# zhiyuan-yang/MILE

Hardware: AMD Instinct MI355X
Metric: MCLMC integrator particle-steps/s (integrator-steps/s x ensemble size) (higher is better)
Workload: dtype f32; 1 GPU; B2: airfoil-shaped N=1052 F=5, FCN hidden_structure [64,64,64,2] relu, Gaussian head, StandardNormal prior, d=8834; ensemble_per_gpu=128, ensemble_total=128, n_thinning=10, integrator=isokinetic McLachlan, O-step-O refresh, 2 full-batch gradients/step, noise=Philox4x32-10 counter RNG, grad_kernel=mfma_w64_bf16x3, parallelism=particles sharded 128/GPU x 1, no collective (one rank, no process group), finite=True

## Files before the change

### mile_amd/csrc/mile_update.h

```cpp
#pragma once
#include <cstdlib>

#include "mile_device.h"

enum : int32_t {
  UPD_FROM_SLABS = 1 << 0,
  UPD_START = 1 << 1,
  UPD_B1 = 1 << 2,
  UPD_OA = 1 << 3,
  UPD_RECORD = 1 << 4,
  UPD_OB = 1 << 5,
  UPD_B2 = 1 << 6,
  UPD_A = 1 << 7,
  UPD_TUNE = 1 << 8,
  UPD_NO_G = 1 << 9,
};

struct UpdParams {
  int32_t d, E, S, flags;
  int32_t dp;
  int32_t prior;
  float prior_loc, prior_scale;
  float *x, *u, *g, *logp;
  const float *slabs, *llpart;
  const float *eps, *L, *sdc;
  const float *zA, *zB;
  uint64_t seed;
  const int32_t *pids;
  uint32_t stepA, stageA, stepB, stageB;
  float coef_b1, coef_b2, coef_a;
  float hA, hB;
  float *dK, *lold;
  float *out_sample;
  float *out_info;
  const float *x_in, *u_in, *g_in, *logp_in;
  float *t_eps;
  float *t_eps_max, *t_time, *t_xavg;
  float *t_W;
  float *t_avg;
  const float *bk_x, *bk_u, *bk_g, *bk_logp;
  float t_mask;
  float t_var;
  float t_trust, t_decay;
  float *upart;
  float *u_rec;
  float *x_acc;
  int32_t force_restart;
  float *nz_A, *nz_B;
  uint32_t nz_stepA, nz_stageA, nz_stepB, nz_stageB;
#ifdef MILE_LAB_UPD_EDGES
  long long *dbg_buf;
#endif
};
#ifdef MILE_LAB_UPD_EDGES
#define UPD_EDGE(k) asm volatile("s_memtime %0\n\ts_waitcnt lgkmcnt(0)" : "=s"(upd_edge[k])::"memory");
#define UPD_EDGE_WAIT asm volatile("s_waitcnt vmcnt(0)" ::: "memory");
#else
#define UPD_EDGE(k)
#define UPD_EDGE_WAIT
#endif

struct Chain {
  float M[4][4];
  float c[4];
  __device__ __forceinline__ float norm() const {
    float s = 0.0f;
#pragma unroll
    for (int a = 0; a < 4; ++a)
#pragma unroll
      for (int b = 0; b < 4; ++b) s = fmaf(c[a] * M[a][b], c[b], s);
    return sqrtf(s);
  }
  __device__ __forceinline__ float B(float eps, float coef, float gnorm, int d) {
    float ue = 0.0f;
#pragma unroll
    for (int a = 0; a < 4; ++a) ue = fmaf(c[a], M[a][1], ue);
    const float delta = eps * coef * gnorm / (float)(d - 1);
    const float omz = -expm1f(-delta);
    const float zeta = 1.0f - omz;
    const float beta = omz * (1.0f + zeta + ue * omz);
#pragma unroll
    for (int a = 0; a < 4; ++a) c[a] *= 2.0f * zeta;
    c[1] += beta;
    const float n = norm();
    if (n > 1e-13f)
#pragma unroll
      for (int a = 0; a < 4; ++a) c[a] /= n;
    return (float)(d - 1) * (delta + log1pf(0.5f * (1.0f - ue) * expm1f(-2.0f * delta)));
  }
  __device__ __forceinline__ void O(int k, float hstep, float L, int d) {
    const float nu = sqrtf(expm1f(2.0f * hstep / L) / (float)d);
    c[k] += nu;
    const float n = norm();
#pragma unroll
    for (int a = 0; a < 4; ++a) c[a] /= n;
  }
};


struct GradNorm {
  float gn, ign, ee;
  bool zero_e;
};
__device__ __forceinline__ GradNorm grad_norm(float gg) {
  GradNorm r;
  r.gn = sqrtf(gg);
  const bool ok = r.gn > 1e-13f;
  r.zero_e = ok && isinf(r.gn);
  r.ign = ok ? 1.0f / r.gn : 1.0f;
  r.ee = ok ? (r.zero_e ? 0.0f : 1.0f) : gg;
  return r;
}
__device__ __forceinline__ void chain_gram(Chain &ch, const float *S, const GradNorm &gnm) {
  const float ig = gnm.ign;
  ch.M[0][0] = S[0]; ch.M[0][1] = gnm.zero_e ? 0.0f : S[1] * ig; ch.M[0][2] = S[3]; ch.M[0][3] = S[6];
  ch.M[1][1] = gnm.ee; ch.M[1][2] = gnm.zero_e ? 0.0f : S[4] * ig; ch.M[1][3] = gnm.zero_e ? 0.0f : S[7] * ig;
  ch.M[2][2] = S[5]; ch.M[2][3] = S[9];
  ch.M[3][3] = S[8];
#pragma unroll
  for (int a = 0; a < 4; ++a)
#pragma unroll
    for (int b = 0; b < 4; ++b)
      if (b < a) ch.M[a][b] = ch.M[b][a];
  ch.c[0] = 1.0f; ch.c[1] = ch.c[2] = ch.c[3] = 0.0f;
}
__device__ __forceinline__ float nan_to_num(float v) {
  constexpr float FMAX = 3.4028234663852886e38f;
  return isnan(v) ? 0.0f : fminf(fmaxf(v, -FMAX), FMAX);
}

#define UPD_NT 1024
#define UPD_NW (UPD_NT / 64)
#define UPD_NSUM 12
#define UPD_QMAX 4

template <bool CACHED>
static __global__ __launch_bounds__(UPD_NT) void k_update(const UpdParams p) {
  __shared__ float red[UPD_NW][UPD_NSUM + 1];
  __shared__ float tot[UPD_NSUM + 1];
  const int tid = threadIdx.x, e = blockIdx.x, d = p.d;
  const size_t base = (size_t)e * d;
  const int nq = (d + 3) >> 2;
  const bool from_slabs = p.flags & UPD_FROM_SLABS;
  const bool useA = p.flags & UPD_OA, useB = p.flags & UPD_OB;
  const uint32_t pid = p.pids ? (uint32_t)p.pids[e] : (uint32_t)e;
  const float *sl = p.slabs + (size_t)e * p.S * p.dp;
  constexpr int NK = CACHED ? UPD_QMAX : 1;
  f32x4 cx[NK], cu[NK], cg[NK], ca[NK], cb[NK];

  float sm[UPD_NSUM];
#pragma unroll
  for (int k = 0; k < UPD_NSUM; ++k) sm[k] = 0.0f;
  auto pass1 = [&](int q, f32x4 &X, f32x4 &U, f32x4 &G, f32x4 &A, f32x4 &B) {
    A = f32x4{0, 0, 0, 0}; B = f32x4{0, 0, 0, 0};
    if (useA && !p.zA) A = philox_normal4(q, pid, p.stepA, p.stageA, p.seed);
    if (useB && !p.zB) B = philox_normal4(q, pid, p.stepB, p.stageB, p.seed);
#pragma unroll
    for (int m = 0; m < 4; ++m) {
      const int i = 4 * q + m;
      X[m] = U[m] = G[m] = 0.0f;
      if (i < d) {
        float gi;
        const float xi = p.x[base + i];
        if (from_slabs) {
          gi = 0.0f;
          for (int s = 0; s < p.S; ++s) gi += sl[(size_t)s * p.dp + i];
          const float t = (xi - p.prior_loc) / p.prior_scale;
          if (p.prior == MILE_PRIOR_NORMAL) {
            gi -= t / p.prior_scale;
            sm[10] = fmaf(-0.5f * t, t, sm[10]);
          } else {
            gi -= (t > 0.0f ? 1.0f : (t < 0.0f ? -1.0f : 0.0f)) / p.prior_scale;
            sm[10] -= fabsf(t);
          }
          p.g[base + i] = gi;
        } else {
          gi = p.g[base + i];
        }
        const float gs = p.sdc ? gi * p.sdc[base + i] : gi;
        const float ui = p.u[base + i];
        if (useA && p.zA) A[m] = p.zA[base + i];
        if (useB && p.zB) B[m] = p.zB[base + i];
        const float a = A[m], b = B[m];
        X[m] = xi; U[m] = ui; G[m] = gs;
        sm[0] = fmaf(ui, ui, sm[0]); sm[1] = fmaf(ui, gs, sm[1]); sm[2] = fmaf(gs, gs, sm[2]);
        sm[3] = fmaf(ui, a, sm[3]); sm[4] = fmaf(gs, a, sm[4]); sm[5] = fmaf(a, a, sm[5]);
        sm[6] = fmaf(ui, b, sm[6]); sm[7] = fmaf(gs, b, sm[7]); sm[8] = fmaf(b, b, sm[8]);
        sm[9] = fmaf(a, b, sm[9]);
      } else {
        A[m] = B[m] = 0.0f;
      }
    }
  };
  if (CACHED) {
#pragma unroll
    for (int k = 0; k < NK; ++k) {
      const int q = tid + k * UPD_NT;
      if (q < nq) pass1(q, cx[k], cu[k], cg[k], ca[k], cb[k]);
    }
  } else {
    for (int q = tid; q < nq; q += UPD_NT) pass1(q, cx[0], cu[0], cg[0], ca[0], cb[0]);
  }
#pragma unroll
  for (int k = 0; k < UPD_NSUM; ++k) sm[k] = wave_sum(sm[k]);
  if ((tid & 63) == 0)
#pragma unroll
    for (int k = 0; k < UPD_NSUM; ++k) red[tid >> 6][k] = sm[k];
  __syncthreads();
  if (tid < UPD_NSUM) {
    float t = 0.0f;
#pragma unroll
    for (int w = 0; w < UPD_NW; ++w) t += red[w][tid];
    tot[tid] = t;
  }
  __syncthreads();

  float S[UPD_NSUM];
#pragma unroll
  for (int k = 0; k < UPD_NSUM; ++k) S[k] = tot[k];
  const float eps = p.eps[e], L = p.L[e];
  float logp_now;
  if (from_slabs) {
    float ll = 0.0f;
    for (int s = 0; s < p.S; ++s) ll += p.llpart[(size_t)e * p.S + s];
    const float cst = p.prior == MILE_PRIOR_NORMAL ? -(float)d * (logf(p.prior_scale) + 0.91893853320467274f)
                                                   : -(float)d * logf(2.0f * p.prior_scale);
    logp_now = ll + (S[10] + cst);
  } else {
    logp_now = p.logp[e];
  }
  const GradNorm gnm = grad_norm(S[2]);
  const float gn = gnm.gn, ign = gnm.ign;
  Chain ch;
  chain_gram(ch, S, gnm);

  float dk = (p.flags & UPD_START) ? 0.0f : p.dK[e];
  float lold = (p.flags & UPD_START) ? logp_now : p.lold[e];
  if (p.flags & UPD_B1) dk += ch.B(eps, p.coef_b1, gn, d);
  if (p.flags & UPD_OA) ch.O(2, p.hA * eps, L, d);
  float info_dk = 0.0f, info_de = 0.0f;
  if (p.flags & UPD_RECORD) {
    info_dk = dk;
    info_de = dk - (logp_now - lold);
    dk = 0.0f;
    lold = logp_now;
  }
  if (p.flags & UPD_OB) ch.O(3, p.hB * eps, L, d);
  if (p.flags & UPD_B2) dk += ch.B(eps, p.coef_b2, gn, d);
  __syncthreads();
  if (tid == 0) {
    p.dK[e] = dk;
    p.lold[e] = lold;
    if (from_slabs) p.logp[e] = logp_now;
    if ((p.flags & UPD_RECORD) && p.out_info) {
      p.out_info[3 * e + 0] = logp_now;
      p.out_info[3 * e + 1] = info_dk;
      p.out_info[3 * e + 2] = info_de;
    }
  }
  const bool any_op = p.flags & (UPD_B1 | UPD_OA | UPD_OB | UPD_B2);
  if (!any_op && !(p.flags & UPD_A) && !p.out_sample) return;

  const float c0 = ch.c[0], c1 = ch.c[1] * ign, c2 = ch.c[2], c3 = ch.c[3];
  const float ea = eps * p.coef_a;
  auto pass2 = [&](int q, const f32x4 &X, const f32x4 &U, const f32x4 &G, const f32x4 &A, const f32x4 &B) {
#pragma unroll
    for (int m = 0; m < 4; ++m) {
      const int i = 4 * q + m;
      if (i < d) {
        const float sd = p.sdc ? p.sdc[base + i] : 1.0f;
        float v = U[m];
        if (any_op) {
          v = fmaf(c0, v, fmaf(c1, G[m], fmaf(c2, A[m], c3 * B[m])));
          p.u[base + i] = v;
        }
        if (p.out_sample) p.out_sample[base + i] = X[m];
        if (p.flags & UPD_A) p.x[base + i] = fmaf(ea * sd, v, X[m]);
      }
    }
  };
  if (CACHED) {
#pragma unroll
    for (int k = 0; k < NK; ++k) {
      const int q = tid + k * UPD_NT;
      if (q < nq) pass2(q, cx[k], cu[k], cg[k], ca[k], cb[k]);
    }
  } else {
    for (int q = tid; q < nq; q += UPD_NT) {
      f32x4 X, U, G, A = {0, 0, 0, 0}, B = {0, 0, 0, 0};
      if (useA && !p.zA) A = philox_normal4(q, pid, p.stepA, p.stageA, p.seed);
      if (useB && !p.zB) B = philox_normal4(q, pid, p.stepB, p.stageB, p.seed);
#pragma unroll
      for (int m = 0; m < 4; ++m) {
        const int i = 4 * q + m;
        X[m] = U[m] = G[m] = 0.0f;
        if (i < d) {
          X[m] = p.x[base + i]; U[m] = p.u[base + i];
          G[m] = p.g[base + i] * (p.sdc ? p.sdc[base + i] : 1.0f);
          if (useA && p.zA) A[m] = p.zA[base + i];
          if (useB && p.zB) B[m] = p.zB[base + i];
        }
      }
      pass2(q, X, U, G, A, B);
    }
  }
}

#define UPD_SEG 8192
template <int PHASE>
static __global__ __launch_bounds__(UPD_NT) void k_update_seg(const UpdParams p, float *upart, int nseg) {
  __shared__ float red[UPD_NW][UPD_NSUM + 1];
  __shared__ float tot[UPD_NSUM + 1];
  const int tid = threadIdx.x, seg = blockIdx.x, e = blockIdx.y, d = p.d;
  const size_t base = (size_t)e * d;
  const int q0 = seg * (UPD_SEG / 4), q1 = min((d + 3) >> 2, q0 + UPD_SEG / 4);
  const bool from_slabs = p.flags & UPD_FROM_SLABS;
  const bool useA = p.flags & UPD_OA, useB = p.flags & UPD_OB;
  const uint32_t pid = p.pids ? (uint32_t)p.pids[e] : (uint32_t)e;
  const float *sl = p.slabs + (size_t)e * p.S * p.dp;
  float *mine = upart + ((size_t)e * nseg + seg) * UPD_NSUM;
  if constexpr (PHASE == 1) {
    float sm[UPD_NSUM];
#pragma unroll
    for (int k = 0; k < UPD_NSUM; ++k) sm[k] = 0.0f;
    for (int q = q0 + tid; q < q1; q += UPD_NT) {
      f32x4 A = {0, 0, 0, 0}, B = {0, 0, 0, 0};
      if (useA && !p.zA) A = philox_normal4(q, pid, p.stepA, p.stageA, p.seed);
      if (useB && !p.zB) B = philox_normal4(q, pid, p.stepB, p.stageB, p.seed);
#pragma unroll
      for (int m = 0; m < 4; ++m) {
        const int i = 4 * q + m;
        if (i < d) {
          float gi;
          const float xi = p.x[base + i];
          if (from_slabs) {
            gi = 0.0f;
            for (int s = 0; s < p.S; ++s) gi += sl[(size_t)s * p.dp + i];
            const float t = (xi - p.prior_loc) / p.prior_scale;
            if (p.prior == MILE_PRIOR_NORMAL) {
              gi -= t / p.prior_scale;
              sm[10] = fmaf(-0.5f * t, t, sm[10]);
            } else {
              gi -= (t > 0.0f ? 1.0f : (t < 0.0f ? -1.0f : 0.0f)) / p.prior_scale;
              sm[10] -= fabsf(t);
            }
            p.g[base + i] = gi;
          } else {
            gi = p.g[base + i];
          }
          const float gs = p.sdc ? gi * p.sdc[base + i] : gi;
          const float ui = p.u[base + i];
          const float a = (useA && p.zA) ? p.zA[base + i] : A[m], b = (useB && p.zB) ? p.zB[base + i] : B[m];
          sm[0] = fmaf(ui, ui, sm[0]); sm[1] = fmaf(ui, gs, sm[1]); sm[2] = fmaf(gs, gs, sm[2]);
          sm[3] = fmaf(ui, a, sm[3]); sm[4] = fmaf(gs, a, sm[4]); sm[5] = fmaf(a, a, sm[5]);
          sm[6] = fmaf(ui, b, sm[6]); sm[7] = fmaf(gs, b, sm[7]); sm[8] = fmaf(b, b, sm[8]);
          sm[9] = fmaf(a, b, sm[9]);
        }
      }
    }
#pragma unroll
    for (int k = 0; k < UPD_NSUM; ++k) sm[k] = wave_sum(sm[k]);
    if ((tid & 63) == 0)
#pragma unroll
      for (int k = 0; k < UPD_NSUM; ++k) red[tid >> 6][k] = sm[k];
    __syncthreads();
    if (tid < UPD_NSUM) {
      float t = 0.0f;
#pragma unroll
      for (int w = 0; w < UPD_NW; ++w) t += red[w][tid];
      mine[tid] = t;
    }
    return;
  } else {
    if (tid < UPD_NSUM) {
      float t = 0.0f;
      for (int sg = 0; sg < nseg; ++sg) t += upart[((size_t)e * nseg + sg) * UPD_NSUM + tid];
      tot[tid] = t;
    }
    __syncthreads();
    float S[UPD_NSUM];
#pragma unroll
    for (int k = 0; k < UPD_NSUM; ++k) S[k] = tot[k];
    const float eps = p.eps[e], L = p.L[e];
    float logp_now;
    if (from_slabs) {
      float ll = 0.0f;
      for (int s = 0; s < p.S; ++s) ll += p.llpart[(size_t)e * p.S + s];
      const float cst = p.prior == MILE_PRIOR_NORMAL ? -(float)d * (logf(p.prior_scale) + 0.91893853320467274f)
                                                     : -(float)d * logf(2.0f * p.prior_scale);
      logp_now = ll + (S[10] + cst);
    } else {
      logp_now = p.logp[e];
    }
    const GradNorm gnm = grad_norm(S[2]);
    const float gn = gnm.gn, ign = gnm.ign;
    Chain ch;
    chain_gram(ch, S, gnm);
    float dk = (p.flags & UPD_START) ? 0.0f : p.dK[e];
    float lold = (p.flags & UPD_START) ? logp_now : p.lold[e];
    if (p.flags & UPD_B1) dk += ch.B(eps, p.coef_b1, gn, d);
    if (p.flags & UPD_OA) ch.O(2, p.hA * eps, L, d);
    float info_dk = 0.0f, info_de = 0.0f;
    if (p.flags & UPD_RECORD) {
      info_dk = dk;
      info_de = dk - (logp_now - lold);
      dk = 0.0f;
      lold = logp_now;
    }
    if (p.flags & UPD_OB) ch.O(3, p.hB * eps, L, d);
    if (p.flags & UPD_B2) dk += ch.B(eps, p.coef_b2, gn, d);
    const bool any_op = p.flags & (UPD_B1 | UPD_OA | UPD_OB | UPD_B2);
    if (seg == 0 && tid == 0) {
      float *st = upart + ((size_t)gridDim.y * nseg) * UPD_NSUM + (size_t)e * 8;
      st[0] = dk; st[1] = lold; st[2] = logp_now; st[3] = info_dk; st[4] = info_de;
    }
    if (!any_op && !(p.flags & UPD_A) && !p.out_sample) return;
    const float c0 = ch.c[0], c1 = ch.c[1] * ign, c2 = ch.c[2], c3 = ch.c[3];
    const float ea = eps * p.coef_a;
    for (int q = q0 + tid; q < q1; q += UPD_NT) {
      f32x4 A = {0, 0, 0, 0}, B = {0, 0, 0, 0};
      if (useA && !p.zA) A = philox_normal4(q, pid, p.stepA, p.stageA, p.seed);
      if (useB && !p.zB) B = philox_normal4(q, pid, p.stepB, p.stageB, p.seed);
#pragma unroll
      for (int m = 0; m < 4; ++m) {
        const int i = 4 * q + m;
        if (i < d) {
          const float sd = p.sdc ? p.sdc[base + i] : 1.0f;
          const float X = p.x[base + i], G = p.g[base + i] * sd;
          const float a = (useA && p.zA) ? p.zA[base + i] : A[m], b = (useB && p.zB) ? p.zB[base + i] : B[m];
          float v = p.u[base + i];
          if (any_op) {
            v = fmaf(c0, v, fmaf(c1, G, fmaf(c2, a, c3 * b)));
            p.u[base + i] = v;
          }
          if (p.out_sample) p.out_sample[base + i] = X;
          if (p.flags & UPD_A) p.x[base + i] = fmaf(ea * sd, v, X);
        }
      }
    }
  }
}
static __global__ __launch_bounds__(256) void k_update_seg_scalars(const UpdParams p, const float *upart, int nseg, int E) {
  const int e = blockIdx.x * 256 + threadIdx.x;
  if (e >= E) return;
  const float *st = upart + ((size_t)E * nseg) * UPD_NSUM + (size_t)e * 8;
  p.dK[e] = st[0];
  p.lold[e] = st[1];
  if (p.flags & UPD_FROM_SLABS) p.logp[e] = st[2];
  if ((p.flags & UPD_RECORD) && p.out_info) {
    p.out_info[3 * e + 0] = st[2];
    p.out_info[3 * e + 1] = st[3];
    p.out_info[3 * e + 2] = st[4];
  }
}

template <int AL>
__device__ __forceinline__ f32x4 ld4(const float *q) {
  if constexpr (AL == 4) {
    return *(const f32x4 *)q;
  } else if constexpr (AL == 2) {
    const f32x2 a = *(const f32x2 *)q, b = *(const f32x2 *)(q + 2);
    return f32x4{a[0], a[1], b[0], b[1]};
  } else {
    return f32x4{q[0], q[1], q[2], q[3]};
  }
}
template <int AL>
__device__ __forceinline__ void st4(float *q, const f32x4 v) {
  if constexpr (AL == 4) {
    *(f32x4 *)q = v;
  } else if constexpr (AL == 2) {
    *(f32x2 *)q = f32x2{v[0], v[1]};
    *(f32x2 *)(q + 2) = f32x2{v[2], v[3]};
  } else {
    q[0] = v[0]; q[1] = v[1]; q[2] = v[2]; q[3] = v[3];
  }
}

typedef uint32_t upd_u32x4 __attribute__((ext_vector_type(4)));
template <int AL, bool COH>
__device__ __forceinline__ f32x4 ld4_slab(const float *row, __amdgpu_buffer_rsrc_t rs, int float_off) {
  if constexpr (COH) {
    return __builtin_bit_cast(f32x4, __builtin_amdgcn_raw_buffer_load_b128(rs, float_off * 4, 0, 16));
  } else {
    return ld4<AL>(row + float_off);
  }
}
template <bool COH>
__device__ __forceinline__ float ld1_shared(const float *q) {
  if constexpr (COH) return __hip_atomic_load(q, __ATOMIC_RELAXED, __HIP_MEMORY_SCOPE_AGENT);
  else return *q;
}

template <int CF>
__host__ __device__ constexpr bool upd_needs(int k) {
  if (CF < 0) return true;
  const bool a = (CF & UPD_OA) != 0, b = (CF & UPD_OB) != 0;
  return k < 3 ? true : k < 6 ? a : k < 9 ? b : k == 9 ? (a && b) : k == 10 ? (CF & UPD_FROM_SLABS) != 0 : (CF & UPD_TUNE) != 0;
}
template <int CF>
__device__ __forceinline__ void upd_add_sums(float (&sm)[UPD_NSUM], float ui, float gs, float a, float b) {
  sm[0] = fmaf(ui, ui, sm[0]); sm[1] = fmaf(ui, gs, sm[1]); sm[2] = fmaf(gs, gs, sm[2]);
  if constexpr (upd_needs<CF>(3)) { sm[3] = fmaf(ui, a, sm[3]); sm[4] = fmaf(gs, a, sm[4]); sm[5] = fmaf(a, a, sm[5]); }
  if constexpr (upd_needs<CF>(6)) { sm[6] = fmaf(ui, b, sm[6]); sm[7] = fmaf(gs, b, sm[7]); sm[8] = fmaf(b, b, sm[8]); }
  if constexpr (upd_needs<CF>(9)) sm[9] = fmaf(a, b, sm[9]);
}

#define UPD_KIND_MID (UPD_FROM_SLABS | UPD_B1 | UPD_A | UPD_NO_G)
#define UPD_KIND_REC (UPD_FROM_SLABS | UPD_B1 | UPD_OA | UPD_RECORD | UPD_OB | UPD_B2 | UPD_A | UPD_NO_G)
#define UPD_KIND_TUNE (UPD_FROM_SLABS | UPD_B1 | UPD_OA | UPD_RECORD | UPD_TUNE | UPD_OB | UPD_B2 | UPD_A)
template <int NK, int AL, bool SDC, bool COH, int CF = -1, bool BIG = false>
__device__ __forceinline__ bool upd_fast_body(const UpdParams &p, const int e, const int tid, const int nt,
                                              float (*red)[UPD_NSUM + 1], float *bc, f32x4 *gl = nullptr) {
  const int d = p.d;
  const int flags = CF >= 0 ? CF : p.flags;
#ifdef MILE_LAB_UPD_EDGES
  unsigned long long upd_edge[10] = {}, upd_rt0, upd_rt1;
  asm volatile("s_memrealtime %0\n\ts_waitcnt lgkmcnt(0)" : "=s"(upd_rt0)::"memory");
#endif
  UPD_EDGE(0)
  const size_t base = (size_t)e * d;
  const int nqf = d >> 2;
  const int ntail = d & 3;
  const bool from_slabs = flags & UPD_FROM_SLABS;
  const bool useA = flags & UPD_OA, useB = flags & UPD_OB;
  const bool explA = useA && p.zA, explB = useB && p.zB;
  const uint32_t pid = p.pids ? (uint32_t)p.pids[e] : (uint32_t)e;
  const float *sl = p.slabs + (size_t)e * p.S * p.dp;
  const __amdgpu_buffer_rsrc_t sl_rs = __builtin_amdgcn_make_buffer_rsrc(const_cast<float *>(sl), 0, p.S * p.dp * 4, 0x00020000);
  const float *xin = p.x_in ? p.x_in : p.x, *uin = p.u_in ? p.u_in : p.u, *gin = p.g_in ? p.g_in : p.g;
  const bool tune = flags & UPD_TUNE;
  const bool merged = tune && p.u_rec != nullptr;
  const bool store_g = from_slabs && !(flags & UPD_NO_G);
  const float ips = 1.0f / p.prior_scale;
  const bool normal = CF >= 0 ? true : p.prior == MILE_PRIOR_NORMAL;

  const float eps_in = p.eps[e], L_in = p.L[e];
  const float dk_in = (flags & UPD_START) ? 0.0f : p.dK[e];
  const float lold_in = (flags & UPD_START) ? 0.0f : p.lold[e];
  const float logp_in = from_slabs ? 0.0f : (p.logp_in ? p.logp_in : p.logp)[e];
  float ll_in = 0.0f;
  if (from_slabs) {
#pragma unroll 8
    for (int s = 0; s < p.S; ++s) ll_in += ld1_shared<COH>(p.llpart + (size_t)e * p.S + s);
  }

  constexpr int NR = BIG ? 1 : NK;
  f32x4 cx[BIG ? 1 : NK], cu[NK], cg[NR], ca[NR], cb[NR], csd[SDC ? NK : 1];
#pragma unroll
  for (int k = 0; k < NK; ++k) {
    const int q = tid + k * nt;
    const bool valid = q < nqf;
    const size_t o = base + 4 * (size_t)(valid ? q : 0);
    if constexpr (!BIG) cx[k] = ld4<AL>(xin + o);
    cu[k] = ld4<AL>(uin + o);
    f32x4 g;
    if (from_slabs) {
      const int so = (int)(o - base);
      g = ld4_slab<AL, COH>(sl, sl_rs, so);
#pragma unroll 4
      for (int s = 1; s < p.S; ++s) g += ld4_slab<AL, COH>(sl, sl_rs, s * p.dp + so);
    } else {
      g = ld4<AL>(gin + o);
    }
    if constexpr (BIG) gl[k * nt + tid] = g;
    else cg[k] = g;
    if constexpr (SDC) csd[k] = ld4<AL>(p.sdc + o);
    if constexpr (!BIG) {
      ca[k] = explA ? ld4<AL>(p.zA + o) : f32x4{0, 0, 0, 0};
      cb[k] = explB ? ld4<AL>(p.zB + o) : f32x4{0, 0, 0, 0};
    }
  }
  const bool has_tail = tid < ntail;
  const size_t to = base + 4 * (size_t)nqf + (has_tail ? tid : 0);
  float tx = 0, tu = 0, tg = 0, ta = 0, tb = 0, tsd = 1.0f;
  if (ntail) {
    const size_t tc = has_tail ? to : base;
    tx = xin[tc]; tu = uin[tc];
    if (from_slabs) {
      tg = 0.0f;
#pragma unroll 4
      for (int s = 0; s < p.S; ++s) tg += ld1_shared<COH>(sl + (size_t)s * p.dp + (tc - base));
    }
    else tg = gin[tc];
    if (SDC) tsd = p.sdc[tc];
    if (explA) ta = p.zA[tc];
    if (explB) tb = p.zB[tc];
  }
  UPD_EDGE(1)
  UPD_EDGE_WAIT
  UPD_EDGE(2)
  float sm[UPD_NSUM];
#pragma unroll
  for (int k = 0; k < UPD_NSUM; ++k) sm[k] = 0.0f;
#pragma unroll
  for (int kq = 0; kq < NK; ++kq) {
    const int q = tid + kq * nt;
    const int k = BIG ? 0 : kq;
    if constexpr (BIG) {
      cx[0] = ld4<AL>(xin + base + (unsigned)(4 * (q < nqf ? q : 0)));
      cg[0] = gl[kq * nt + tid];
      ca[0] = f32x4{0, 0, 0, 0};
      cb[0] = f32x4{0, 0, 0, 0};
    }
    if (useA && !p.zA) ca[k] = philox_normal4(q, pid, p.stepA, p.stageA, p.seed);
    if (useB && !p.zB) cb[k] = philox_normal4(q, pid, p.stepB, p.stageB, p.seed);
    const float mk = q < nqf ? 1.0f : 0.0f;
#pragma unroll
    for (int m = 0; m < 4; ++m) {
      float gi = cg[k][m];
      const float xi = cx[k][m];
      if (from_slabs) {
        const float t = (xi - p.prior_loc) * ips;
        if (normal) { gi = fmaf(-t, ips, gi); sm[10] = fmaf(-0.5f * mk * t, t, sm[10]); }
        else { gi -= (t > 0.0f ? ips : (t < 0.0f ? -ips : 0.0f)); sm[10] -= mk * fabsf(t); }
      }
      cg[k][m] = gi;
      if (tune) sm[11] += (mk != 0.0f && !isfinite(xi)) ? 1.0f : 0.0f;
      const float gs = (SDC ? gi * csd[kq][m] : gi) * mk;
      const float ui = cu[kq][m] * mk, a = ca[k][m] * mk, b = cb[k][m] * mk;
      ca[k][m] = a; cb[k][m] = b;
      upd_add_sums<CF>(sm, ui, gs, a, b);
    }
    if (store_g && q < nqf) {
      f32x4 gst = cg[k];
      if (tune) {
#pragma unroll
        for (int m = 0; m < 4; ++m) gst[m] = nan_to_num(gst[m]);
      }
      st4<AL>(p.g + base + 4 * (size_t)q, gst);
    }
    if constexpr (SDC) {
#pragma unroll
      for (int m = 0; m < 4; ++m) cg[k][m] *= csd[kq][m];
    }
    if constexpr (BIG) {
      gl[kq * nt + tid] = cg[0];
      __builtin_amdgcn_sched_barrier(0);
    }
  }
  if (ntail) {
    f32x4 za = {0, 0, 0, 0}, zb = {0, 0, 0, 0};
    if (useA && !p.zA) za = philox_normal4(nqf, pid, p.stepA, p.stageA, p.seed);
    if (useB && !p.zB) zb = philox_normal4(nqf, pid, p.stepB, p.stageB, p.seed);
    const int t = has_tail ? tid : 0;
    if (useA && !p.zA) ta = za[t];
    if (useB && !p.zB) tb = zb[t];
    const float mk = has_tail ? 1.0f : 0.0f;
    if (from_slabs) {
      const float tt = (tx - p.prior_loc) * ips;
      if (normal) { tg = fmaf(-tt, ips, tg); sm[10] = fmaf(-0.5f * mk * tt, tt, sm[10]); }
      else { tg -= (tt > 0.0f ? ips : (tt < 0.0f ? -ips : 0.0f)); sm[10] -= mk * fabsf(tt); }
      if (has_tail && store_g) p.g[to] = tune ? nan_to_num(tg) : tg;
    }
    if (tune) sm[11] += (has_tail && !isfinite(tx)) ? 1.0f : 0.0f;
    tg *= tsd;
    const float gs = tg * mk, ui = tu * mk;
    ta *= mk; tb *= mk;
    upd_add_sums<CF>(sm, ui, gs, ta, tb);
  }
  UPD_EDGE(3)
#pragma unroll
  for (int k = 0; k < UPD_NSUM; ++k)
    if (upd_needs<CF>(k)) sm[k] = wave_sum(sm[k]);
  if ((tid & 63) == 0)
#pragma unroll
    for (int k = 0; k < UPD_NSUM; ++k)
      if (upd_needs<CF>(k)) red[tid >> 6][k] = sm[k];
  UPD_EDGE(4)
  __syncthreads();
  UPD_EDGE(5)

  if (tid < 64) {
  float S[UPD_NSUM];
  {
    float t = 0.0f;
    const int kk = tid < UPD_NSUM ? tid : 0;
#pragma unroll
    for (int w = 0; w < (nt >> 6); ++w) t += red[w][kk];
#pragma unroll
    for (int k = 0; k < UPD_NSUM; ++k)
      S[k] = upd_needs<CF>(k) ? __builtin_bit_cast(float, __builtin_amdgcn_readlane(__builtin_bit_cast(int, t), k)) : 0.0f;
  }
  const float eps = eps_in, L = L_in;
  float logp_now;
  if (from_slabs) {
    const float ll = ll_in;
    const float cst = normal ? -(float)d * (logf(p.prior_scale) + 0.91893853320467274f)
                             : -(float)d * logf(2.0f * p.prior_scale);
    logp_now = ll + (S[10] + cst);
  } else {
    logp_now = logp_in;
  }
  const GradNorm gnm = grad_norm(S[2]);
  const float gn = gnm.gn, ign = gnm.ign;
  Chain ch;
  chain_gram(ch, S, gnm);
  float dk = (flags & UPD_START) ? 0.0f : dk_in;
  float lold = (flags & UPD_START) ? logp_now : lold_in;
  if (flags & UPD_B1) dk += ch.B(eps, p.coef_b1, gn, d);
  if (flags & UPD_OA) ch.O(2, p.hA * eps, L, d);
  float info_dk = 0.0f, info_de = 0.0f;
  if (flags & UPD_RECORD) {
    info_dk = dk;
    info_de = dk - (logp_now - lold);
    dk = 0.0f;
    lold = logp_now;
  }
  bool t_ok = true;
  float t_wgt = 0.0f, t_Wold = 0.0f;
  float eps_next = eps;
  const float r0 = ch.c[0], r1 = ch.c[1] * ign, r2 = ch.c[2], r3 = ch.c[3];
  bool t_simple = true;
  if (tune) {
    constexpr float FMAX = 3.4028234663852886e38f;
    t_ok = S[11] == 0.0f;
    float dE = info_de;
    dE = t_ok ? (isnan(dE) ? 0.0f : fminf(fmaxf(dE, -FMAX), FMAX)) : 0.0f;
    const float emax_old = p.t_eps_max[e];
    const float emax = t_ok ? nan_to_num(emax_old) : 0.8f * eps;
    const float xi = dE * dE / ((float)d * p.t_var) + 1e-8f;
    const float lx = logf(xi) / (6.0f * p.t_trust);
    const float w = expf(-0.5f * lx * lx);
    const float e2 = eps * eps;
    const float xavg = p.t_decay * p.t_xavg[e] + w * (xi / (e2 * e2 * e2));
    const float tm = p.t_decay * p.t_time[e] + w;
    float en = powf(xavg / tm, -1.0f / 6.0f);
    en = (en < emax ? 1.0f : 0.0f) * en + (en > emax ? 1.0f : 0.0f) * emax;
    t_Wold = p.t_W[e];
    t_wgt = (1.0f - p.t_mask) * (t_ok ? 1.0f : 0.0f) * en;
    logp_now = t_ok ? nan_to_num(logp_now) : p.bk_logp[e];
    eps_next = en;
    t_simple = t_ok && isfinite(S[2]) && isfinite(S[0]) && isfinite(r0) && isfinite(r1) && isfinite(r2) && isfinite(r3) &&
               !p.force_restart;
    if (merged) lold = logp_now;
    if (tid == 0) {
      p.t_eps[e] = en;
      p.t_eps_max[e] = emax;
      p.t_xavg[e] = xavg;
      p.t_time[e] = tm;
      p.t_W[e] = t_Wold + t_wgt;
    }
  }
  if (flags & UPD_OB) ch.O(3, p.hB * eps_next, L, d);
  if (flags & UPD_B2) dk += ch.B(eps_next, p.coef_b2, gn, d);
  if (tid == 0) {
    p.dK[e] = dk;
    p.lold[e] = lold;
    if (from_slabs || tune) p.logp[e] = logp_now;
    if ((flags & UPD_RECORD) && p.out_info) {
      p.out_info[3 * e + 0] = logp_now;
      p.out_info[3 * e + 1] = info_dk;
      p.out_info[3 * e + 2] = info_de;
    }
    bc[0] = ch.c[0]; bc[1] = ch.c[1] * ign; bc[2] = ch.c[2]; bc[3] = ch.c[3];
    bc[4] = eps_next * p.coef_a; bc[5] = t_ok ? 1.0f : 0.0f; bc[6] = t_Wold; bc[7] = t_wgt;
    if (merged) { bc[8] = r0; bc[9] = r1; bc[10] = r2; bc[11] = r3; bc[12] = t_simple ? 1.0f : 0.0f; }
  }
  }
  UPD_EDGE(6)
  __syncthreads();
  UPD_EDGE(7)
  const bool any_op = flags & (UPD_B1 | UPD_OA | UPD_OB | UPD_B2);
  const bool doA = flags & UPD_A;
  const float c0 = bc[0], c1 = bc[1], c2 = bc[2], c3 = bc[3], ea = bc[4];
  const bool t_ok = bc[5] != 0.0f;
  const float t_Wold = bc[6], t_wgt = bc[7];
  if (tune && !t_ok) {
    float *xo = merged ? p.x_acc : p.x, *uo = merged ? p.u_rec : p.u;
    for (int i = tid; i < d; i += nt) {
      xo[base + i] = p.bk_x[base + i];
      uo[base + i] = p.bk_u[base + i];
      p.g[base + i] = p.bk_g[base + i];
    }
    return merged;
  }
  float rc0 = 0.0f, rc1 = 0.0f, rc2 = 0.0f;
  bool simple = true;
  if (merged) { rc0 = bc[8]; rc1 = bc[9]; rc2 = bc[10]; simple = bc[12] != 0.0f; }
  const bool t_acc = tune && p.t_mask == 0.0f;
  const float t_den = 1.0f / (t_Wold + t_wgt);
#pragma unroll
  for (int kq = 0; kq < NK; ++kq) {
    const int q = tid + kq * nt;
    const int k = BIG ? 0 : kq;
    if (q < nqf) {
      const size_t o = base + 4 * (size_t)q;
      if constexpr (BIG) {
        cx[0] = ld4<AL>(xin + base + (unsigned)(4 * q));
        cg[0] = gl[kq * nt + tid];
        if (flags & (UPD_OA | UPD_OB)) {
          ca[0] = f32x4{0, 0, 0, 0};
          cb[0] = f32x4{0, 0, 0, 0};
          int q2 = q;
          asm volatile("" : "+v"(q2));
          if (useA && !p.zA) ca[0] = philox_normal4(q2, pid, p.stepA, p.stageA, p.seed);
          if (useB && !p.zB) cb[0] = philox_normal4(q2, pid, p.stepB, p.stageB, p.seed);
        } else {
          ca[0] = f32x4{0, 0, 0, 0}; cb[0] = f32x4{0, 0, 0, 0};
        }
      }
      if (t_acc) {
        float *a0 = p.t_avg + (size_t)e * 2 * d + 4 * (size_t)q, *a1 = a0 + d;
        f32x4 m0 = ld4<AL>(a0), m1 = ld4<AL>(a1);
#pragma unroll
        for (int m = 0; m < 4; ++m) {
          m0[m] = (t_Wold * m0[m] + t_wgt * cx[k][m]) * t_den;
          m1[m] = (t_Wold * m1[m] + t_wgt * cx[k][m] * cx[k][m]) * t_den;
        }
        st4<AL>(a0, m0);
        st4<AL>(a1, m1);
      }
      f32x4 v = cu[kq];
      if (merged) {
        f32x4 ur;
#pragma unroll
        for (int m = 0; m < 4; ++m) ur[m] = nan_to_num(fmaf(rc0, cu[kq][m], fmaf(rc1, cg[k][m], rc2 * ca[k][m])));
        st4<AL>(p.u_rec + o, ur);
        if (!simple) continue;
      }
      if (any_op) {
#pragma unroll
        for (int m = 0; m < 4; ++m) v[m] = fmaf(c0, cu[kq][m], fmaf(c1, cg[k][m], fmaf(c2, ca[k][m], c3 * cb[k][m])));
        if (tune && !merged) {
#pragma unroll
          for (int m = 0; m < 4; ++m) v[m] = nan_to_num(v[m]);
        }
        st4<AL>(p.u + o, v);
      }
      if (p.out_sample) st4<AL>(p.out_sample + o, cx[k]);
      if (doA) {
        f32x4 xn;
#pragma unroll
        for (int m = 0; m < 4; ++m) xn[m] = fmaf(SDC ? ea * csd[kq][m] : ea, v[m], cx[k][m]);
        st4<AL>(p.x + o, xn);
      }
    }
    if constexpr (BIG) __builtin_amdgcn_sched_barrier(0);
  }
  if (has_tail) {
    if (t_acc) {
      float *a0 = p.t_avg + (size_t)e * 2 * d + 4 * (size_t)nqf + tid, *a1 = a0 + d;
      *a0 = (t_Wold * *a0 + t_wgt * tx) * t_den;
      *a1 = (t_Wold * *a1 + t_wgt * tx * tx) * t_den;
    }
    float v = tu;
    if (merged) p.u_rec[to] = nan_to_num(fmaf(rc0, tu, fmaf(rc1, tg, rc2 * ta)));
    if (!merged || simple) {
      if (any_op) { v = fmaf(c0, tu, fmaf(c1, tg, fmaf(c2, ta, c3 * tb))); if (tune && !merged) v = nan_to_num(v); p.u[to] = v; }
      if (p.out_sample) p.out_sample[to] = tx;
      if (doA) p.x[to] = fmaf(ea * tsd, v, tx);
    }
  }
#ifdef MILE_LAB_UPD_EDGES
  UPD_EDGE(8)
  UPD_EDGE_WAIT
  UPD_EDGE(9)
  asm volatile("s_memrealtime %0\n\ts_waitcnt lgkmcnt(0)" : "=s"(upd_rt1)::"memory");
  if (e == 0 && tid == 0 && p.dbg_buf) {
#pragma unroll
    for (int k = 1; k < 10; ++k) p.dbg_buf[k] += (long long)(upd_edge[k] - upd_edge[0]);
    p.dbg_buf[0] += 1;
    p.dbg_buf[10] += (long long)(upd_rt1 - upd_rt0);
  }
#endif
  return merged && !simple;
}

template <int NK, int AL, bool SDC>
__device__ __forceinline__ void upd_tune_restart(const UpdParams &p, const int e, const int tid, const int nt,
                                                 float (*red)[UPD_NSUM + 1], float *bc) {
  __syncthreads();
  UpdParams q = p;
  q.flags = UPD_START | UPD_B2 | UPD_A | (p.flags & UPD_OB);
  q.x_in = p.x_acc; q.u_in = p.u_rec; q.g_in = p.g; q.logp_in = p.logp;
  q.eps = p.t_eps;
  q.u_rec = nullptr; q.x_acc = nullptr; q.out_info = nullptr; q.out_sample = nullptr; q.zA = nullptr;
  upd_fast_body<NK, AL, SDC, false, -1>(q, e, tid, nt, red, bc);
}

template <int NK, int AL>
__device__ __forceinline__ void upd_noise_body(const UpdParams &p, const int e, const int tid, const int nt) {
  const int d = p.d, nqf = d >> 2, ntail = d & 3;
  const size_t base = (size_t)e * d;
  const uint32_t pid = p.pids ? (uint32_t)p.pids[e] : (uint32_t)e;
#pragma unroll
  for (int k = 0; k < NK; ++k) {
    const int q = tid + k * nt;
    if (q < nqf) {
      if (p.nz_A) st4<AL>(p.nz_A + base + 4 * (size_t)q, philox_normal4(q, pid, p.nz_stepA, p.nz_stageA, p.seed));
      if (p.nz_B) st4<AL>(p.nz_B + base + 4 * (size_t)q, philox_normal4(q, pid, p.nz_stepB, p.nz_stageB, p.seed));
    }
  }
  if (ntail && tid == 0) {
    const size_t o = base + 4 * (size_t)nqf;
    if (p.nz_A) {
      const f32x4 z = philox_normal4(nqf, pid, p.nz_stepA, p.nz_stageA, p.seed);
      for (int t = 0; t < ntail; ++t) p.nz_A[o + t] = z[t];
    }
    if (p.nz_B) {
      const f32x4 z = philox_normal4(nqf, pid, p.nz_stepB, p.nz_stageB, p.seed);
      for (int t = 0; t < ntail; ++t) p.nz_B[o + t] = z[t];
    }
  }
}

template <int NK, int AL, bool SDC, int CF = -1, int MAXT = UPD_NT>
static __global__ __launch_bounds__(MAXT) void k_update_fast(const UpdParams p) {
  __shared__ float red[UPD_NW][UPD_NSUM + 1];
  __shared__ float bc[16];
  if constexpr (CF == UPD_KIND_MID) {
    if ((int)blockIdx.x >= p.E) {
#ifdef MILE_LAB_UPD_EDGES
      unsigned long long upd_edge[2];
      UPD_EDGE(0)
#endif
      upd_noise_body<NK, AL>(p, blockIdx.x - p.E, threadIdx.x, blockDim.x);
#ifdef MILE_LAB_UPD_EDGES
      UPD_EDGE_WAIT
      UPD_EDGE(1)
      if ((int)blockIdx.x == p.E && threadIdx.x == 0 && p.dbg_buf) p.dbg_buf[16] += (long long)(upd_edge[1] - upd_edge[0]);
#endif
      return;
    }
  }
  const bool again = upd_fast_body<NK, AL, SDC, false, CF>(p, blockIdx.x, threadIdx.x, blockDim.x, red, bc);
  if constexpr (CF < 0 || (CF & UPD_TUNE) != 0) {
    if (again) upd_tune_restart<NK, AL, SDC>(p, blockIdx.x, threadIdx.x, blockDim.x, red, bc);
  }
}

#define UPD_QMAX_BIG 9
template <int NK, int AL, bool SDC, int CF = -1>
static __global__ __launch_bounds__(UPD_NT) void k_update_big(const UpdParams p) {
  __shared__ float red[UPD_NW][UPD_NSUM + 1];
  __shared__ float bc[16];
  extern __shared__ __attribute__((aligned(16))) char upd_gl[];
  upd_fast_body<NK, AL, SDC, false, CF, true>(p, blockIdx.x, threadIdx.x, blockDim.x, red, bc, reinterpret_cast<f32x4 *>(upd_gl));
}

static inline int upd_kind(const UpdParams &u) {
  if (u.prior != MILE_PRIOR_NORMAL || u.sdc) return -1;
  if (u.flags == UPD_KIND_MID) return UPD_KIND_MID;
  if (u.flags == UPD_KIND_REC) return UPD_KIND_REC;
  if (u.flags == UPD_KIND_TUNE && u.u_rec) return UPD_KIND_TUNE;
  return -1;
}

static inline bool upd_fast_d(int d) { return (d >> 2) >= 1 && (d >> 2) <= UPD_NT * UPD_QMAX; }

#define AUX_NT 256
__device__ __forceinline__ float slab_grad_logprior(const float *sl, int S, int dp, int i, int prior, float loc, float scale,
                                                    float theta_i, float &pv) {
  float gi = 0.0f;
  for (int s = 0; s < S; ++s) gi += sl[(size_t)s * dp + i];
  const float t = (theta_i - loc) / scale;
  if (prior == MILE_PRIOR_NORMAL) { gi -= t / scale; pv += -0.5f * t * t; }
  else { gi -= (t > 0.0f ? 1.0f : (t < 0.0f ? -1.0f : 0.0f)) / scale; pv += -fabsf(t); }
  return gi;
}
__device__ __forceinline__ double llpart_logprior(const float *llpart, int S, int e, int d, int prior, float scale, double pv) {
  double t = pv;
  for (int s = 0; s < S; ++s) t += (double)llpart[(size_t)e * S + s];
  t += prior == MILE_PRIOR_NORMAL ? -(double)d * (log((double)scale) + 0.91893853320467274)
                                  : -(double)d * log(2.0 * (double)scale);
  return t;
}

static __global__ __launch_bounds__(AUX_NT) void k_finalize(int d, int dp, int S, int prior, float loc, float scale,
                                                     const float *theta, const float *slabs,
                                                     const float *llpart, float *grad, float *logp) {
  __shared__ float red[AUX_NT / 64];
  const int tid = threadIdx.x, e = blockIdx.x;
  const size_t base = (size_t)e * d;
  const float *sl = slabs + (size_t)e * S * dp;
  float pv = 0.0f;
  for (int i = tid; i < d; i += AUX_NT) grad[base + i] = slab_grad_logprior(sl, S, dp, i, prior, loc, scale, theta[base + i], pv);
  pv = wave_sum(pv);
  if ((tid & 63) == 0) red[tid >> 6] = pv;
  __syncthreads();
  if (tid == 0) {
    double t = 0.0;
    for (int w = 0; w < AUX_NT / 64; ++w) t += (double)red[w];
    logp[e] = (float)llpart_logprior(llpart, S, e, d, prior, scale, t);
  }
}

static __global__ __launch_bounds__(AUX_NT) void k_init_momentum(int d, const float *z, uint64_t seed,
                                                          const int32_t *pids, float *u) {
  __shared__ float red[AUX_NT / 64];
  const int tid = threadIdx.x, e = blockIdx.x;
  const size_t base = (size_t)e * d;
  const uint32_t pid = pids ? (uint32_t)pids[e] : (uint32_t)e;
  const int nq = (d + 3) >> 2;
  float ss = 0.0f;
  for (int q = tid; q < nq; q += AUX_NT) {
    f32x4 zz = {0, 0, 0, 0};
    if (!z) zz = philox_normal4(q, pid, 0u, 2u, seed);
#pragma unroll
    for (int m = 0; m < 4; ++m) {
      const int i = 4 * q + m;
      if (i < d) {
        const float v = z ? z[base + i] : zz[m];
        u[base + i] = v;
        ss = fmaf(v, v, ss);
      }
    }
  }
  ss = wave_sum(ss);
  if ((tid & 63) == 0) red[tid >> 6] = ss;
  __syncthreads();
  float t = 0.0f;
  for (int w = 0; w < AUX_NT / 64; ++w) t += red[w];
  const float inv = 1.0f / sqrtf(t);
  for (int i = tid; i < d; i += AUX_NT) u[base + i] *= inv;
}

static __global__ __launch_bounds__(AUX_NT) void k_debug_noise(int d, uint64_t seed, const int32_t *pids,
                                                        uint32_t step, uint32_t stage, float *out) {
  const int tid = threadIdx.x, e = blockIdx.x;
  const uint32_t pid = pids ? (uint32_t)pids[e] : (uint32_t)e;
  const int nq = (d + 3) >> 2;
  for (int q = tid; q < nq; q += AUX_NT) {
    const f32x4 zz = philox_normal4(q, pid, step, stage, seed);
    for (int m = 0; m < 4; ++m)
      if (4 * q + m < d) out[(size_t)e * d + 4 * q + m] = zz[m];
  }
}

struct TunePostParams {
  int32_t d;
  float *x, *u, *g, *logp;
  const float *bk_x, *bk_u, *bk_g, *bk_logp;
  float *info;
  float *t_eps, *t_eps_max, *t_time, *t_xavg, *t_W, *t_avg;
  float t_mask, t_var, t_trust, t_decay;
};

static __global__ __launch_bounds__(AUX_NT) void k_tune_post(const TunePostParams p) {
  __shared__ float red[AUX_NT / 64];
  __shared__ float bc[4];
  const int tid = threadIdx.x, e = blockIdx.x, d = p.d;
  const size_t base = (size_t)e * d;
  __shared__ float red2[AUX_NT / 64];
  float bad = 0.0f, bad_ug = 0.0f;
  for (int i = tid; i < d; i += AUX_NT) {
    bad += isfinite(p.x[base + i]) ? 0.0f : 1.0f;
    bad_ug += (isfinite(p.u[base + i]) && isfinite(p.g[base + i])) ? 0.0f : 1.0f;
  }
  bad = wave_sum(bad);
  bad_ug = wave_sum(bad_ug);
  if ((tid & 63) == 0) { red[tid >> 6] = bad; red2[tid >> 6] = bad_ug; }
  __syncthreads();
  if (tid == 0) {
    constexpr float FMAX = 3.4028234663852886e38f;
    float cnt = 0.0f;
    for (int w = 0; w < AUX_NT / 64; ++w) cnt += red[w];
    const bool ok = cnt == 0.0f;
    const float eps = p.t_eps[e];
    float dE = p.info[3 * e + 2];
    dE = ok ? (isnan(dE) ? 0.0f : fminf(fmaxf(dE, -FMAX), FMAX)) : 0.0f;
    const float emax = ok ? nan_to_num(p.t_eps_max[e]) : 0.8f * eps;
    const float xi = dE * dE / ((float)d * p.t_var) + 1e-8f;
    const float lx = logf(xi) / (6.0f * p.t_trust);
    const float w = expf(-0.5f * lx * lx);
    const float e2 = eps * eps;
    const float xavg = p.t_decay * p.t_xavg[e] + w * (xi / (e2 * e2 * e2));
    const float tm = p.t_decay * p.t_time[e] + w;
    float en = powf(xavg / tm, -1.0f / 6.0f);
    en = (en < emax ? 1.0f : 0.0f) * en + (en > emax ? 1.0f : 0.0f) * emax;
    const float Wold = p.t_W[e], wgt = (1.0f - p.t_mask) * (ok ? 1.0f : 0.0f) * en;
    p.t_eps[e] = en; p.t_eps_max[e] = emax; p.t_xavg[e] = xavg; p.t_time[e] = tm; p.t_W[e] = Wold + wgt;
    if (!ok) { p.logp[e] = p.bk_logp[e]; p.info[3 * e] = p.bk_logp[e]; }
    else p.logp[e] = nan_to_num(p.logp[e]);
    float cug = 0.0f;
    for (int w = 0; w < AUX_NT / 64; ++w) cug += red2[w];
    bc[0] = ok ? 1.0f : 0.0f; bc[1] = Wold; bc[2] = wgt; bc[3] = cug;
  }
  __syncthreads();
  const bool ok = bc[0] != 0.0f;
  if (!ok) {
    for (int i = tid; i < d; i += AUX_NT) {
      p.x[base + i] = p.bk_x[base + i];
      p.u[base + i] = p.bk_u[base + i];
      p.g[base + i] = p.bk_g[base + i];
    }
    return;
  }
  if (bc[3] != 0.0f)
    for (int i = tid; i < d; i += AUX_NT) {
      p.u[base + i] = nan_to_num(p.u[base + i]);
      p.g[base + i] = nan_to_num(p.g[base + i]);
    }
  if (p.t_mask == 0.0f) {
    const float Wold = bc[1], wgt = bc[2], den = 1.0f / (Wold + wgt);
    float *a0 = p.t_avg + (size_t)e * 2 * d, *a1 = a0 + d;
    for (int i = tid; i < d; i += AUX_NT) {
      const float xv = p.x[base + i];
      a0[i] = (Wold * a0[i] + wgt * xv) * den;
      a1[i] = (Wold * a1[i] + wgt * xv * xv) * den;
    }
  }
}

struct OptimParams {
  int32_t d, S, dp, kind;
  float lr, b1, b2, eps, wd, inv_batch;
  float bc1, bc2;
  float *theta, *m, *v;
  const float *slabs, *llpart;
  const uint8_t *active;
  float *out_nll;
};
static __global__ __launch_bounds__(256) void k_optim_step(const OptimParams p) {
  const int e = blockIdx.y;
  const int i = blockIdx.x * 256 + threadIdx.x;
  if (blockIdx.x == 0 && threadIdx.x == 0 && p.out_nll) {
    float ll = 0.0f;
    for (int s = 0; s < p.S; ++s) ll += p.llpart[(size_t)e * p.S + s];
    p.out_nll[e] = -ll * p.inv_batch;
  }
  if (i >= p.d) return;
  if (p.active && !p.active[e]) return;
  const float *sl = p.slabs + (size_t)e * p.S * p.dp + i;
  float g = 0.0f;
#pragma unroll 4
  for (int s = 0; s < p.S; ++s) g += sl[(size_t)s * p.dp];
  g = -g * p.inv_batch;
  const size_t o = (size_t)e * p.d + i;
  const float th = p.theta[o];
  float upd;
  if (p.kind == MILE_OPT_SGD) {
    upd = p.lr * g;
  } else {
    const float m = p.b1 * p.m[o] + (1.0f - p.b1) * g;
    const float v = p.b2 * p.v[o] + (1.0f - p.b2) * g * g;
    p.m[o] = m; p.v[o] = v;
    const float mh = m / p.bc1, vh = v / p.bc2;
    upd = p.lr * (mh / (sqrtf(vh) + p.eps) + (p.kind == MILE_OPT_ADAMW ? p.wd * th : 0.0f));
  }
  p.theta[o] = th - upd;
}
```

Baseline: 975,300 particle-steps/s.

## Spread per-particle chain scalar math across wave-0 lanes and defer energy bookkeeping

Result: no change. 981,400 particle-steps/s, median of 6 (+0.6%).

```diff
diff --git a/mile_amd/csrc/mile_update.h b/mile_amd/csrc/mile_update.h
--- a/mile_amd/csrc/mile_update.h
+++ b/mile_amd/csrc/mile_update.h
@@ -509,6 +509,121 @@
 #define UPD_KIND_MID (UPD_FROM_SLABS | UPD_B1 | UPD_A | UPD_NO_G)
 #define UPD_KIND_REC (UPD_FROM_SLABS | UPD_B1 | UPD_OA | UPD_RECORD | UPD_OB | UPD_B2 | UPD_A | UPD_NO_G)
 #define UPD_KIND_TUNE (UPD_FROM_SLABS | UPD_B1 | UPD_OA | UPD_RECORD | UPD_TUNE | UPD_OB | UPD_B2 | UPD_A)
+
+__device__ __forceinline__ float upd_lane(float v, int k) {
+  return __builtin_bit_cast(float, __builtin_amdgcn_readlane(__builtin_bit_cast(int, v), k));
+}
+struct ChainPre { float nuA, nuB, lcst; };
+struct ChainLate { float ue1, dl1, em21, ue2, dl2, em22, logp_now; };
+
+template <int CF>
+__device__ __forceinline__ ChainPre chain_pre(const UpdParams &p, const int lane, const float eps, const float L, const int d) {
+#pragma clang fp contract(off)
+  ChainPre r{0.0f, 0.0f, 0.0f};
+  r.lcst = logf(p.prior_scale) + 0.91893853320467274f;
+  if constexpr ((CF & (UPD_OA | UPD_OB)) != 0) {
+    const float h = (lane & 1) ? p.hB : p.hA;
+    const float nu = sqrtf(expm1f(2.0f * (h * eps) / L) / (float)d);
+    r.nuA = upd_lane(nu, 0);
+    r.nuB = upd_lane(nu, 1);
+  }
+  return r;
+}
+
+template <int CF>
+__device__ __forceinline__ ChainLate chain_lanes(const UpdParams &p, const int lane, const int nt, float (*red)[UPD_NSUM + 1],
+                                                 float *bc, const ChainPre &pre, const float eps, const float ll, const int d) {
+#pragma clang fp contract(off)
+  constexpr bool REC = CF == UPD_KIND_REC;
+  float S[UPD_NSUM];
+  {
+    float t = 0.0f;
+    const int kk = lane < UPD_NSUM ? lane : 0;
+#pragma unroll
+    for (int w = 0; w < (nt >> 6); ++w) t += red[w][kk];
+#pragma unroll
+    for (int k = 0; k < UPD_NSUM; ++k) S[k] = upd_needs<CF>(k) ? upd_lane(t, k) : 0.0f;
+  }
+  ChainLate o{};
+  o.logp_now = upd_lane(ll + fmaf(-pre.lcst, (float)d, S[10]), 0);
+  const GradNorm gnm = grad_norm(S[2]);
+  Chain ch;
+  chain_gram(ch, S, gnm);
+  const float coef = (REC && lane >= 2) ? p.coef_b2 : p.coef_b1;
+  const float dl = eps * coef * gnm.gn / (float)(d - 1);
+  const float em = expm1f((lane & 1) ? -2.0f * dl : -dl);
+  o.dl1 = upd_lane(dl, 0); o.em21 = upd_lane(em, 1);
+  if constexpr (REC) { o.dl2 = upd_lane(dl, 2); o.em22 = upd_lane(em, 3); }
+
+  float cl = 0.0f;
+  auto normalise = [&](bool guarded) {
+    const float n = ch.norm();
+    cl = lane == 0 ? ch.c[0] : lane == 1 ? ch.c[1] : lane == 2 ? ch.c[2] : ch.c[3];
+    if (!guarded || n > 1e-13f) cl /= n;
+  };
+  auto gather = [&]() {
+#pragma unroll
+    for (int a = 0; a < 4; ++a) ch.c[a] = upd_lane(cl, a);
+  };
+  auto Bstep = [&](const float em1) {
+    float ue = 0.0f;
+#pragma unroll
+    for (int a = 0; a < 4; ++a) ue = fmaf(ch.c[a], ch.M[a][1], ue);
+    const float omz = -em1;
+    const float zeta = 1.0f - omz;
+    const float beta = omz * fmaf(ue, omz, 1.0f + zeta);
+    const float tz = 2.0f * zeta;
+#pragma unroll
+    for (int a = 0; a < 4; ++a) ch.c[a] *= tz;
+    ch.c[1] += beta;
+    normalise(true);
+    return upd_lane(ue, 0);
+  };
+  o.ue1 = Bstep(upd_lane(em, 0));
+  if constexpr (REC) {
+    gather();
+    ch.c[2] += pre.nuA;
+    normalise(false);
+    gather();
+    ch.c[3] += pre.nuB;
+    normalise(false);
+    gather();
+    o.ue2 = Bstep(upd_lane(em, 2));
+  }
+  const float out = lane == 1 ? cl * gnm.ign : lane == 4 ? eps * p.coef_a : cl;
+  if (lane < 5) bc[lane] = out;
+  return o;
+}
+
+template <int CF>
+__device__ __forceinline__ void chain_energy(const UpdParams &p, const int e, const int lane, const ChainLate &o,
+                                             const float dk_in, const float lold_in, const int d) {
+#pragma clang fp contract(off)
+  constexpr bool REC = CF == UPD_KIND_REC;
+  const bool second = REC && (lane & 1);
+  const float ue = second ? o.ue2 : o.ue1, dl = second ? o.dl2 : o.dl1, em2 = second ? o.em22 : o.em21;
+  const float en = dl + log1pf(0.5f * (1.0f - ue) * em2);
+  const float dm1 = (float)(d - 1);
+  float dk = fmaf(dm1, upd_lane(en, 0), dk_in), lold = lold_in;
+  float info_dk = 0.0f, info_de = 0.0f;
+  if constexpr (REC) {
+    info_dk = dk;
+    info_de = dk - (o.logp_now - lold);
+    lold = o.logp_now;
+    dk = fmaf(dm1, upd_lane(en, 1), 0.0f);
+  }
+  if (lane == 0) {
+    p.dK[e] = dk;
+    p.lold[e] = lold;
+    p.logp[e] = o.logp_now;
+    if (REC && p.out_info) {
+      p.out_info[3 * e + 0] = o.logp_now;
+      p.out_info[3 * e + 1] = info_dk;
+      p.out_info[3 * e + 2] = info_de;
+    }
+  }
+}
+
 template <int NK, int AL, bool SDC, bool COH, int CF = -1, bool BIG = false>
 __device__ __forceinline__ bool upd_fast_body(const UpdParams &p, const int e, const int tid, const int nt,
                                               float (*red)[UPD_NSUM + 1], float *bc, f32x4 *gl = nullptr) {
@@ -668,10 +783,15 @@
     for (int k = 0; k < UPD_NSUM; ++k)
       if (upd_needs<CF>(k)) red[tid >> 6][k] = sm[k];
   UPD_EDGE(4)
+  constexpr bool LANES = CF == UPD_KIND_MID || CF == UPD_KIND_REC;
+  [[maybe_unused]] const bool wave0 = LANES && __builtin_amdgcn_readfirstlane(tid) < 64;
+  [[maybe_unused]] ChainLate late{};
   __syncthreads();
   UPD_EDGE(5)
 
-  if (tid < 64) {
+  if constexpr (LANES) {
+    if (wave0) late = chain_lanes<CF>(p, tid, nt, red, bc, chain_pre<CF>(p, tid, eps_in, L_in, d), eps_in, ll_in, d);
+  } else if (tid < 64) {
   float S[UPD_NSUM];
   {
     float t = 0.0f;
@@ -852,8 +972,12 @@
       if (doA) p.x[to] = fmaf(ea * tsd, v, tx);
     }
   }
+  UPD_EDGE(8)
+  if constexpr (LANES) {
+    __builtin_amdgcn_sched_barrier(0);
+    if (wave0) chain_energy<CF>(p, e, tid, late, dk_in, lold_in, d);
+  }
 #ifdef MILE_LAB_UPD_EDGES
-  UPD_EDGE(8)
   UPD_EDGE_WAIT
   UPD_EDGE(9)
   asm volatile("s_memrealtime %0\n\ts_waitcnt lgkmcnt(0)" : "=s"(upd_rt1)::"memory");
```
